# JADGardner/neusky

Measured on AMD Instinct MI355X. Metric: train rays/sec on NeRF-OSR lk2 @1024 rays x 96 samples, higher is better.
Workload: dtype f32 in memory; forward products: fp16 hi + residual split, 3 x v_mfma_f32_32x32x16_f16 per product on power-of-two pre-scaled operands, one fp32 accumulator (~2^-22): FiLM-SIREN chains and the SDF / albedo field alike; backward products: the same fp16 split on per-row / per-matrix pre-scaled gradien; 1 GPU; full NeuSky train step (BASELINE configs[2]): 1024 rays/GPU x 96 samples, proposal 256+96, 512 illumination directions (256 upper-hemisphere DDF queries/ray), illumination decoder = this project's FiLM-SIREN H = 128 (RENI-shaped: latent 100x3; the reference's configured Attention decoder is absent from its tree), hash L16 F2 T2^19 x2, 256-wide MLPs; fwd + losses + bwd + all-reduce + 5 Adam groups; rays_per_gpu=1024, samples_per_ray=96, illumination_directions=512, parallelism=ray-sharded dp1, launcher=self-spawned, launch=HIP graph replay (1 graph/step + all-reduce + 5 Adam launches)

## Files before the change

### neusky_amd/csrc/wgrad_native.hip

```cpp
#include "common.h"
#include "../../include/neusky_hip.h"

namespace {

typedef _Float16 f16x8 __attribute__((ext_vector_type(8)));
typedef float f32x16 __attribute__((ext_vector_type(16)));
typedef float f32x4 __attribute__((ext_vector_type(4)));
typedef short s16x4 __attribute__((__vector_size__(4 * sizeof(short))));
typedef __attribute__((address_space(3))) s16x4 lds_s16x4;

struct WgradProblem {
  const float* A;
  const float* B;
  float* dW;
  float* db;
  const float* a_scale_max;
  float b_scale;
  const float* b_scale_max;
  int nnt_a, nnt_b, ldw;
  int tile0;
  int lda, ldb;
  int wa, wb;
  int bias_rows;
  int bias_mod;
};
struct WgradArgs {
  WgradProblem p[NSKY_WGRAD_MAX_PROBLEMS];
  int n_problems, rows, row_blocks, blocks_per_split, n_tiles;
};

__device__ __forceinline__ float pow2_scale(float m, float& inv) {
  if (!(m > 0.0f) || !(m < 3.0e38f)) { inv = 1.0f; return 1.0f; }
  int e;
  (void)frexpf(m, &e);
  e = max(-100, min(100, e));
  inv = ldexpf(1.0f, e - 15);
  return ldexpf(1.0f, 15 - e);
}

__device__ __forceinline__ int xcd_contiguous(int id, int total) {
  const int xcd = id & 7, idx = id >> 3, per = total >> 3, rem = total & 7;
  return xcd * per + min(xcd, rem) + idx;
}

template <bool BF>
__device__ __forceinline__ f32x16 mma(f16x8 x, f16x8 y, f32x16 acc) {
  typedef __bf16 b16x8 __attribute__((ext_vector_type(8)));
  if (BF) return __builtin_amdgcn_mfma_f32_32x32x16_bf16(__builtin_bit_cast(b16x8, x), __builtin_bit_cast(b16x8, y), acc, 0, 0, 0);
  return __builtin_amdgcn_mfma_f32_32x32x16_f16(x, y, acc, 0, 0, 0);
}

template <int WM, int WN, int TM, int TN, bool RM>
__global__ __launch_bounds__(64 * WM * WN, WM * WN == 8 ? 1 : 2) void wgrad_native_kernel(WgradArgs a) {
  constexpr int NW = WM * WN;
  constexpr int NT = NW;
  static_assert(WM * TM == NT && WN * TN == NT, "square output block");
  constexpr int OPB = NT * 4096;
  constexpr int STAGE = 2 * OPB;
  extern __shared__ __attribute__((aligned(16))) unsigned char smem[];

  const int tid = threadIdx.x, lane = tid & 63, wave = tid >> 6;
  const int wm = wave / WN, wn = wave % WN;
  const int logical = xcd_contiguous(blockIdx.x, gridDim.x);
  const int gtile = logical % a.n_tiles, split = logical / a.n_tiles;
  int pi = 0;
  while (pi + 1 < a.n_problems && gtile >= a.p[pi + 1].tile0) ++pi;
  const WgradProblem& P = a.p[pi];
  const int tile = gtile - P.tile0;
  const int kblocks = P.nnt_b / NT;
  const int nb = tile / kblocks, kb = tile % kblocks;
  const int r_beg = split * a.blocks_per_split;
  const int r_end = min(a.row_blocks, r_beg + a.blocks_per_split);
  if (r_beg >= r_end) return;

  float a_inv = 1.0f;
  const float a_scale = P.a_scale_max ? pow2_scale(*P.a_scale_max, a_inv) : 1.0f;
  float b_unused;
  const float b_scale = P.b_scale_max ? pow2_scale(*P.b_scale_max, b_unused) : P.b_scale;
  const bool clamp_b = P.b_scale_max == nullptr;

  const int c = lane & 31, hh = lane >> 5;
  const int rq = lane >> 3, fq = lane & 7;
  const int fa = (nb * NT + wave) * 32 + 4 * fq, fb = (kb * NT + wave) * 32 + 4 * fq;
  const bool fa_ok = fa < P.wa, fb_ok = fb < P.wb;
  const float* pa = RM ? P.A + (long)r_beg * 32 * P.lda + min(fa, max(P.wa - 4, 0))
                       : P.A + ((long)r_beg * P.nnt_a + nb * NT + wave) * 1024 + lane * 4;
  const float* pb = RM ? P.B + (long)r_beg * 32 * P.ldb + min(fb, max(P.wb - 4, 0))
                       : P.B + ((long)r_beg * P.nnt_b + kb * NT + wave) * 1024 + lane * 4;
  const long a_step = RM ? 32l * P.lda : (long)P.nnt_a * 1024, b_step = RM ? 32l * P.ldb : (long)P.nnt_b * 1024;
  int rm_row0 = 0;
  f32x4 raw[8];
  const float* pa2 = pa;
  const float* pb2 = pb;
  auto reload = [&](int uu) {
    if (RM) {
      const int row = min(rm_row0 + 8 * (uu >> 1) + rq, a.rows - 1) - rm_row0;
      raw[uu] = __builtin_nontemporal_load(reinterpret_cast<const f32x4*>(((uu & 1) ? pb2 + (long)row * P.ldb : pa2 + (long)row * P.lda)));
    } else {
      raw[uu] = __builtin_nontemporal_load(reinterpret_cast<const f32x4*>(((uu & 1) ? pb2 : pa2) + (uu >> 1) * 256));
    }
  };
  float bias[4][4];
#pragma unroll
  for (int u = 0; u < 4; ++u)
#pragma unroll
    for (int i = 0; i < 4; ++i) bias[u][i] = 0.0f;
  const bool want_bias = P.db != nullptr && kb == 0;
  const int w_base = wave * 4096 + c * 64 + 8 * hh;
  const int w_swz = (c >> 1) & 3;
  typedef _Float16 f16x4 __attribute__((ext_vector_type(4)));
  typedef __bf16 b16x4 __attribute__((ext_vector_type(4)));
  auto stage_unit = [&](int uu, int row0, bool row_block_live, unsigned char* stage) {
    const int op = uu & 1, u = uu >> 1;
    const float s = op == 0 ? a_scale : b_scale;
    const int row = row0 + (RM ? 8 * u + rq : c);
    const bool live = row_block_live && row < a.rows && (!RM || (op == 0 ? fa_ok : fb_ok));
    const bool bias_on = op == 0 && row < P.bias_rows && (P.bias_mod <= 1 || (row % P.bias_mod) == 0);
    float v[4];
#pragma unroll
    for (int i = 0; i < 4; ++i) {
      v[i] = live ? raw[uu][i] * s : 0.0f;
      if (op == 1 && clamp_b) v[i] = __builtin_amdgcn_fmed3f(v[i], -65504.0f, 65504.0f);
      if (op == 0) bias[u][i] += bias_on ? v[i] : 0.0f;
    }
    unsigned char* img;
    if (RM) {
      const int r = 8 * u + rq;
      img = stage + op * OPB + wave * 4096 + r * 64 + 16 * ((fq >> 1) ^ ((r >> 1) & 3)) + 8 * (fq & 1);
      b16x4 h4, l4;
#pragma unroll
      for (int i = 0; i < 4; ++i) { h4[i] = (__bf16)v[i]; l4[i] = (__bf16)(v[i] - (float)h4[i]); }
      *reinterpret_cast<b16x4*>(img) = h4;
      *reinterpret_cast<b16x4*>(img + 2048) = l4;
    } else {
      img = stage + op * OPB + w_base + 16 * (u ^ w_swz);
      f16x4 h4, l4;
#pragma unroll
      for (int i = 0; i < 4; ++i) { h4[i] = (_Float16)v[i]; l4[i] = (_Float16)(v[i] - (float)h4[i]); }
      *reinterpret_cast<f16x4*>(img) = h4;
      *reinterpret_cast<f16x4*>(img + 2048) = l4;
    }
  };

  const int i16 = lane & 15, q = i16 >> 2, p = i16 & 3, gsel = (lane >> 4) & 1, h = lane >> 5;
  int t_off[2];
#pragma unroll
  for (int rd = 0; rd < 2; ++rd) {
    const int row = 8 * h + 4 * rd + q;
    t_off[rd] = row * 64 + 16 * ((2 * gsel + (p >> 1)) ^ ((row >> 1) & 3)) + 8 * (p & 1);
  }
  auto frag = [&](const unsigned char* img, int ks) -> f16x8 {
    const s16x4 lo4 = __builtin_amdgcn_ds_read_tr16_b64_v4i16((lds_s16x4*)(img + ks * 1024 + t_off[0]));
    const s16x4 hi4 = __builtin_amdgcn_ds_read_tr16_b64_v4i16((lds_s16x4*)(img + ks * 1024 + t_off[1]));
    typedef short s16x8 __attribute__((ext_vector_type(8)));
    const s16x8 v = {lo4[0], lo4[1], lo4[2], lo4[3], hi4[0], hi4[1], hi4[2], hi4[3]};
    return __builtin_bit_cast(f16x8, v);
  };

  f32x16 acc[TM][TN];
#pragma unroll
  for (int i = 0; i < TM; ++i)
#pragma unroll
    for (int j = 0; j < TN; ++j)
#pragma unroll
      for (int r = 0; r < 16; ++r) acc[i][j][r] = 0.0f;

  rm_row0 = r_beg * 32;
#pragma unroll
  for (int uu = 0; uu < 8; ++uu) reload(uu);
  {
    if (r_beg + 1 < r_end) { pa2 += a_step; pb2 += b_step; rm_row0 += 32; }
#pragma unroll
    for (int uu = 0; uu < 8; ++uu) {
      stage_unit(uu, r_beg * 32, true, smem);
      reload(uu);
    }
    if (r_beg + 2 < r_end) { pa2 += a_step; pb2 += b_step; rm_row0 += 32; }
  }
  static_assert(TN == 4 || TN == 2, "one staging unit per (k-step, X tile) point, or two");
  constexpr int UPP = 8 / (2 * TN);
  int cur = 0;
  for (int r = r_beg; r < r_end; ++r) {
    __syncthreads();
    const bool live = r + 1 < r_end;
    const unsigned char* st = smem + cur * STAGE;
    unsigned char* nxt = smem + (cur ^ 1) * STAGE;
#pragma unroll
    for (int ks = 0; ks < 2; ++ks) {
      f16x8 ah[TM], al[TM], bh[2], bl[2];
#pragma unroll
      for (int i = 0; i < TM; ++i) {
        ah[i] = frag(st + (wm * TM + i) * 4096, ks);
        al[i] = frag(st + (wm * TM + i) * 4096 + 2048, ks);
      }
      bh[0] = frag(st + OPB + (wn * TN) * 4096, ks);
      bl[0] = frag(st + OPB + (wn * TN) * 4096 + 2048, ks);
#pragma unroll
      for (int j = 0; j < TN; ++j) {
        if (j + 1 < TN) {
          bh[(j + 1) & 1] = frag(st + OPB + (wn * TN + j + 1) * 4096, ks);
          bl[(j + 1) & 1] = frag(st + OPB + (wn * TN + j + 1) * 4096 + 2048, ks);
        }
#pragma unroll
        for (int i = 0; i < TM; ++i) acc[i][j] = mma<RM>(al[i], bh[j & 1], acc[i][j]);
#pragma unroll
        for (int i = 0; i < TM; ++i) acc[i][j] = mma<RM>(ah[i], bl[j & 1], acc[i][j]);
#pragma unroll
        for (int i = 0; i < TM; ++i) acc[i][j] = mma<RM>(ah[i], bh[j & 1], acc[i][j]);
#pragma unroll
        for (int k = 0; k < UPP; ++k) {
          const int uu = (ks * TN + j) * UPP + k;
          stage_unit(uu, (r + 1) * 32, live, nxt);
          reload(uu);
        }
        __builtin_amdgcn_sched_barrier(0);
      }
    }
    if (r + 3 < r_end) { pa2 += a_step; pb2 += b_step; rm_row0 += 32; }
    cur ^= 1;
  }

  const float out_scale = a_inv / b_scale;
  const int n0 = (nb * NT + wm * TM) * 32, k0 = (kb * NT + wn * TN) * 32;
#pragma unroll
  for (int i = 0; i < TM; ++i)
#pragma unroll
    for (int j = 0; j < TN; ++j) {
      float* out = P.dW + (long)(n0 + 32 * i + 4 * h) * P.ldw + k0 + 32 * j + (lane & 31);
      const bool col_ok = k0 + 32 * j + (lane & 31) < P.wb;
#pragma unroll
      for (int g = 0; g < 16; ++g)
        if (col_ok && n0 + 32 * i + 4 * h + 8 * (g >> 2) + (g & 3) < P.wa)
          atomicAdd(out + (long)(8 * (g >> 2) + (g & 3)) * P.ldw, acc[i][j][g] * out_scale);
      __builtin_amdgcn_sched_barrier(0);
    }
  if (want_bias && RM) {
#pragma unroll
    for (int i = 0; i < 4; ++i) {
      float v = (bias[0][i] + bias[1][i]) + (bias[2][i] + bias[3][i]);
#pragma unroll
      for (int off = 8; off < 64; off <<= 1) v += __shfl_xor(v, off, 64);
      if (rq == 0 && fa + i < P.wa) atomicAdd(P.db + fa + i, v * a_inv);
    }
  } else if (want_bias) {
#pragma unroll
    for (int u = 0; u < 4; ++u)
#pragma unroll
      for (int i = 0; i < 4; ++i) {
        float v = bias[u][i];
#pragma unroll
        for (int off = 16; off > 0; off >>= 1) v += __shfl_xor(v, off, 64);
        if (c == 0 && (nb * NT + wave) * 32 + 8 * u + 4 * hh + i < P.wa) atomicAdd(P.db + (nb * NT + wave) * 32 + 8 * u + 4 * hh + i, v * a_inv);
      }
  }
}

}

extern "C" int nsky_wgrad_native_batch(const nsky_wgrad_problem* problems, int32_t n_problems, int32_t rows, nsky_stream_t stream) {
  NSKY_CHECK_ARG(problems && n_problems >= 1 && n_problems <= NSKY_WGRAD_MAX_PROBLEMS && rows >= 0,
                 "nsky_wgrad_native_batch: 1..%d problems expected, got %d", NSKY_WGRAD_MAX_PROBLEMS, n_problems);
  if (rows == 0) return NSKY_OK;
  WgradArgs a;
  const bool rm = problems[0].lda > 0;
  bool wide = true;
  for (int i = 0; i < n_problems; ++i) {
    const nsky_wgrad_problem& q = problems[i];
    NSKY_CHECK_ARG(q.dZ && q.X && q.dW, "nsky_wgrad_native_batch: problem %d: null argument", i);
    NSKY_CHECK_ARG((q.lda > 0) == rm && (q.ldb > 0) == rm, "nsky_wgrad_native_batch: problem %d: row-major and tile-native operands in one launch", i);
    if (rm) {
      NSKY_CHECK_ARG(q.width_a >= 4 && q.width_b >= 4 && q.width_a % 4 == 0 && q.width_b % 4 == 0 && q.lda >= q.width_a && q.ldb >= q.width_b &&
                         q.lda % 4 == 0 && q.ldb % 4 == 0, "nsky_wgrad_native_batch: problem %d: row-major widths / leading dimensions must be multiples of 4", i);
      NSKY_CHECK_ARG(q.ldw >= q.width_b && q.a_scale_max == nullptr, "nsky_wgrad_native_batch: problem %d: ldw %d < %d, or a scale with row-major operands", i,
                     q.ldw, q.width_b);
      wide = wide && q.width_a > 128 && q.width_b > 128;
    } else {
      NSKY_CHECK_ARG(q.nnt_a > 0 && q.nnt_b > 0 && q.nnt_a % 4 == 0 && q.nnt_b % 4 == 0,
                     "nsky_wgrad_native_batch: problem %d: both operands need a multiple of 128 features (got %d and %d tiles of 32)", i,
                     q.nnt_a, q.nnt_b);
      NSKY_CHECK_ARG(q.width_a >= 0 && q.width_a <= 32 * q.nnt_a && q.width_b >= 0 && q.width_b <= 32 * q.nnt_b,
                     "nsky_wgrad_native_batch: problem %d: widths %d / %d exceed the tiles", i, q.width_a, q.width_b);
      NSKY_CHECK_ARG(q.ldw >= (q.width_b > 0 ? q.width_b : 32 * q.nnt_b), "nsky_wgrad_native_batch: problem %d: ldw %d too small", i, q.ldw);
      int e = 0;
      NSKY_CHECK_ARG(q.b_scale > 0.0f && frexpf(q.b_scale, &e) == 0.5f, "nsky_wgrad_native_batch: problem %d: b_scale must be a power of two", i);
      wide = wide && q.nnt_a % 8 == 0 && q.nnt_b % 8 == 0;
    }
  }
  const int NT = wide ? 8 : 4;
  int tiles = 0;
  for (int i = 0; i < n_problems; ++i) {
    const nsky_wgrad_problem& q = problems[i];
    WgradProblem& P = a.p[i];
    P.A = q.dZ; P.B = q.X; P.dW = q.dW; P.db = q.db; P.a_scale_max = q.a_scale_max; P.b_scale = rm ? 1.0f : q.b_scale;
    P.b_scale_max = rm ? nullptr : q.b_scale_max;
    P.nnt_a = rm ? ceil_div(q.width_a, 32 * NT) * NT : q.nnt_a;
    P.nnt_b = rm ? ceil_div(q.width_b, 32 * NT) * NT : q.nnt_b;
    P.ldw = q.ldw; P.tile0 = tiles;
    P.lda = q.lda; P.ldb = q.ldb;
    P.wa = (rm || q.width_a > 0) ? q.width_a : 32 * q.nnt_a;
    P.wb = (rm || q.width_b > 0) ? q.width_b : 32 * q.nnt_b;
    P.bias_rows = q.bias_rows > 0 ? q.bias_rows : rows;
    P.bias_mod = rm ? 0 : q.bias_row_mod;
    tiles += (P.nnt_a / NT) * (P.nnt_b / NT);
  }
  a.n_problems = n_problems; a.rows = rows; a.n_tiles = tiles;
  a.row_blocks = ceil_div(rows, 32);
  const int slots = wide ? 256 : 512;
  int splits = slots / a.n_tiles;
  if (splits < 1) splits = 1;
  if (splits > a.row_blocks) splits = a.row_blocks;
  a.blocks_per_split = ceil_div(a.row_blocks, splits);
  splits = ceil_div(a.row_blocks, a.blocks_per_split);
  const dim3 grid(a.n_tiles * splits);
  const size_t smem = 2 * 2 * NT * 4096;
  static bool attr_set = [] {
    (void)hipFuncSetAttribute(reinterpret_cast<const void*>(&wgrad_native_kernel<4, 2, 2, 4, false>), hipFuncAttributeMaxDynamicSharedMemorySize, 160 * 1024);
    (void)hipFuncSetAttribute(reinterpret_cast<const void*>(&wgrad_native_kernel<2, 2, 2, 2, false>), hipFuncAttributeMaxDynamicSharedMemorySize, 160 * 1024);
    (void)hipFuncSetAttribute(reinterpret_cast<const void*>(&wgrad_native_kernel<4, 2, 2, 4, true>), hipFuncAttributeMaxDynamicSharedMemorySize, 160 * 1024);
    (void)hipFuncSetAttribute(reinterpret_cast<const void*>(&wgrad_native_kernel<2, 2, 2, 2, true>), hipFuncAttributeMaxDynamicSharedMemorySize, 160 * 1024);
    return true;
  }();
  (void)attr_set;
  const hipStream_t st = (hipStream_t)stream;
  if (wide && rm) hipLaunchKernelGGL((wgrad_native_kernel<4, 2, 2, 4, true>), grid, dim3(512), smem, st, a);
  else if (wide) hipLaunchKernelGGL((wgrad_native_kernel<4, 2, 2, 4, false>), grid, dim3(512), smem, st, a);
  else if (rm) hipLaunchKernelGGL((wgrad_native_kernel<2, 2, 2, 2, true>), grid, dim3(256), smem, st, a);
  else hipLaunchKernelGGL((wgrad_native_kernel<2, 2, 2, 2, false>), grid, dim3(256), smem, st, a);
  NSKY_CHECK_LAUNCH("nsky_wgrad_native_batch");
  return NSKY_OK;
}

extern "C" int nsky_wgrad_native(const float* dZ, int32_t nnt_a, const float* X, int32_t nnt_b, int32_t rows, float* dW, int32_t ldw,
                                 float* db, const float* a_scale_max, float b_scale, nsky_stream_t stream) {
  nsky_wgrad_problem q = {};
  q.dZ = dZ; q.nnt_a = nnt_a; q.X = X; q.nnt_b = nnt_b; q.dW = dW; q.ldw = ldw; q.db = db; q.a_scale_max = a_scale_max; q.b_scale = b_scale;
  return nsky_wgrad_native_batch(&q, 1, rows, stream);
}
```

Before: 52410 rays/s.

## Triple-buffer wgrad LDS per k-step and prefetch next fragments across barriers

Splits the per-row-block LDS staging into half-block (16-row k-step) slots arranged as a three-slot ring, reducing LDS use from 2x to 1.5x of a full block. Fragments for the next k-step are read from LDS during the last MFMA group of the current step, so LDS reads overlap the matrix math. The global-load lane mapping and bias reduction are reorganised to match the new layout. This adds one barrier per k-step, where there was one per row block, and holds more fragment registers live, in exchange for hiding LDS read latency.

```diff
diff --git a/neusky_amd/csrc/wgrad_native.hip b/neusky_amd/csrc/wgrad_native.hip
--- a/neusky_amd/csrc/wgrad_native.hip
+++ b/neusky_amd/csrc/wgrad_native.hip
@@ -55,8 +55,8 @@
   constexpr int NW = WM * WN;
   constexpr int NT = NW;
   static_assert(WM * TM == NT && WN * TN == NT, "square output block");
-  constexpr int OPB = NT * 4096;
-  constexpr int STAGE = 2 * OPB;
+  constexpr int OPB = NT * 2048;
+  constexpr int SLOT = 2 * OPB;
   extern __shared__ __attribute__((aligned(16))) unsigned char smem[];
 
   const int tid = threadIdx.x, lane = tid & 63, wave = tid >> 6;
@@ -79,66 +79,68 @@
   const float b_scale = P.b_scale_max ? pow2_scale(*P.b_scale_max, b_unused) : P.b_scale;
   const bool clamp_b = P.b_scale_max == nullptr;
 
-  const int c = lane & 31, hh = lane >> 5;
+  const int kr = (lane & 7) + 8 * ((lane >> 4) & 1), hh = (lane >> 3) & 1, ug = lane >> 5;
   const int rq = lane >> 3, fq = lane & 7;
   const int fa = (nb * NT + wave) * 32 + 4 * fq, fb = (kb * NT + wave) * 32 + 4 * fq;
   const bool fa_ok = fa < P.wa, fb_ok = fb < P.wb;
+  const int lane_off = ug * 256 + hh * 128 + kr * 4;
   const float* pa = RM ? P.A + (long)r_beg * 32 * P.lda + min(fa, max(P.wa - 4, 0))
-                       : P.A + ((long)r_beg * P.nnt_a + nb * NT + wave) * 1024 + lane * 4;
+                       : P.A + ((long)r_beg * P.nnt_a + nb * NT + wave) * 1024 + lane_off;
   const float* pb = RM ? P.B + (long)r_beg * 32 * P.ldb + min(fb, max(P.wb - 4, 0))
-                       : P.B + ((long)r_beg * P.nnt_b + kb * NT + wave) * 1024 + lane * 4;
+                       : P.B + ((long)r_beg * P.nnt_b + kb * NT + wave) * 1024 + lane_off;
   const long a_step = RM ? 32l * P.lda : (long)P.nnt_a * 1024, b_step = RM ? 32l * P.ldb : (long)P.nnt_b * 1024;
   int rm_row0 = 0;
   f32x4 raw[8];
   const float* pa2 = pa;
   const float* pb2 = pb;
   auto reload = [&](int uu) {
+    const int ks = uu >> 2, v = (uu >> 1) & 1, op = uu & 1;
     if (RM) {
-      const int row = min(rm_row0 + 8 * (uu >> 1) + rq, a.rows - 1) - rm_row0;
-      raw[uu] = __builtin_nontemporal_load(reinterpret_cast<const f32x4*>(((uu & 1) ? pb2 + (long)row * P.ldb : pa2 + (long)row * P.lda)));
+      const int row = min(rm_row0 + 16 * ks + 8 * v + rq, a.rows - 1) - rm_row0;
+      raw[uu] = __builtin_nontemporal_load(reinterpret_cast<const f32x4*>((op ? pb2 + (long)row * P.ldb : pa2 + (long)row * P.lda)));
     } else {
-      raw[uu] = __builtin_nontemporal_load(reinterpret_cast<const f32x4*>(((uu & 1) ? pb2 : pa2) + (uu >> 1) * 256));
+      raw[uu] = __builtin_nontemporal_load(reinterpret_cast<const f32x4*>((op ? pb2 : pa2) + v * 512 + ks * 64));
     }
   };
-  float bias[4][4];
-#pragma unroll
-  for (int u = 0; u < 4; ++u)
-#pragma unroll
-    for (int i = 0; i < 4; ++i) bias[u][i] = 0.0f;
+  float bias[2][4];
+#pragma unroll
+  for (int v = 0; v < 2; ++v)
+#pragma unroll
+    for (int i = 0; i < 4; ++i) bias[v][i] = 0.0f;
   const bool want_bias = P.db != nullptr && kb == 0;
-  const int w_base = wave * 4096 + c * 64 + 8 * hh;
-  const int w_swz = (c >> 1) & 3;
+  const int bias_rows = P.bias_rows, bias_mod = max(P.bias_mod, 1);
+  const bool mod_by_lane = 16 % bias_mod == 0;
+  const bool lane_mod_ok = (RM ? rq : kr) % bias_mod == 0;
   typedef _Float16 f16x4 __attribute__((ext_vector_type(4)));
   typedef __bf16 b16x4 __attribute__((ext_vector_type(4)));
-  auto stage_unit = [&](int uu, int row0, bool row_block_live, unsigned char* stage) {
-    const int op = uu & 1, u = uu >> 1;
+  auto stage_unit = [&](int uu, int row0, bool row_block_live, unsigned char* slot) {
+    const int ks = uu >> 2, v = (uu >> 1) & 1, op = uu & 1;
     const float s = op == 0 ? a_scale : b_scale;
-    const int row = row0 + (RM ? 8 * u + rq : c);
+    const int kro = RM ? 8 * v + rq : kr;
+    const int row = row0 + 16 * ks + kro;
     const bool live = row_block_live && row < a.rows && (!RM || (op == 0 ? fa_ok : fb_ok));
-    const bool bias_on = op == 0 && row < P.bias_rows && (P.bias_mod <= 1 || (row % P.bias_mod) == 0);
-    float v[4];
+    const bool bias_on = op == 0 && row < bias_rows && (mod_by_lane ? lane_mod_ok : row % bias_mod == 0);
+    float x[4];
 #pragma unroll
     for (int i = 0; i < 4; ++i) {
-      v[i] = live ? raw[uu][i] * s : 0.0f;
-      if (op == 1 && clamp_b) v[i] = __builtin_amdgcn_fmed3f(v[i], -65504.0f, 65504.0f);
-      if (op == 0) bias[u][i] += bias_on ? v[i] : 0.0f;
-    }
-    unsigned char* img;
+      x[i] = live ? raw[uu][i] * s : 0.0f;
+      if (op == 1 && clamp_b) x[i] = __builtin_amdgcn_fmed3f(x[i], -65504.0f, 65504.0f);
+      if (op == 0) bias[v][i] += bias_on ? x[i] : 0.0f;
+    }
+    unsigned char* img = slot + op * OPB + wave * 2048 + kro * 64 + 8 * (RM ? (fq & 1) : hh) +
+                         16 * ((RM ? fq >> 1 : 2 * v + ug) ^ ((kro >> 1) & 3));
     if (RM) {
-      const int r = 8 * u + rq;
-      img = stage + op * OPB + wave * 4096 + r * 64 + 16 * ((fq >> 1) ^ ((r >> 1) & 3)) + 8 * (fq & 1);
       b16x4 h4, l4;
 #pragma unroll
-      for (int i = 0; i < 4; ++i) { h4[i] = (__bf16)v[i]; l4[i] = (__bf16)(v[i] - (float)h4[i]); }
+      for (int i = 0; i < 4; ++i) { h4[i] = (__bf16)x[i]; l4[i] = (__bf16)(x[i] - (float)h4[i]); }
       *reinterpret_cast<b16x4*>(img) = h4;
-      *reinterpret_cast<b16x4*>(img + 2048) = l4;
+      *reinterpret_cast<b16x4*>(img + 1024) = l4;
     } else {
-      img = stage + op * OPB + w_base + 16 * (u ^ w_swz);
       f16x4 h4, l4;
 #pragma unroll
-      for (int i = 0; i < 4; ++i) { h4[i] = (_Float16)v[i]; l4[i] = (_Float16)(v[i] - (float)h4[i]); }
+      for (int i = 0; i < 4; ++i) { h4[i] = (_Float16)x[i]; l4[i] = (_Float16)(x[i] - (float)h4[i]); }
       *reinterpret_cast<f16x4*>(img) = h4;
-      *reinterpret_cast<f16x4*>(img + 2048) = l4;
+      *reinterpret_cast<f16x4*>(img + 1024) = l4;
     }
   };
 
@@ -149,9 +151,9 @@
     const int row = 8 * h + 4 * rd + q;
     t_off[rd] = row * 64 + 16 * ((2 * gsel + (p >> 1)) ^ ((row >> 1) & 3)) + 8 * (p & 1);
   }
-  auto frag = [&](const unsigned char* img, int ks) -> f16x8 {
-    const s16x4 lo4 = __builtin_amdgcn_ds_read_tr16_b64_v4i16((lds_s16x4*)(img + ks * 1024 + t_off[0]));
-    const s16x4 hi4 = __builtin_amdgcn_ds_read_tr16_b64_v4i16((lds_s16x4*)(img + ks * 1024 + t_off[1]));
+  auto frag = [&](const unsigned char* img) -> f16x8 {
+    const s16x4 lo4 = __builtin_amdgcn_ds_read_tr16_b64_v4i16((lds_s16x4*)(img + t_off[0]));
+    const s16x4 hi4 = __builtin_amdgcn_ds_read_tr16_b64_v4i16((lds_s16x4*)(img + t_off[1]));
     typedef short s16x8 __attribute__((ext_vector_type(8)));
     const s16x8 v = {lo4[0], lo4[1], lo4[2], lo4[3], hi4[0], hi4[1], hi4[2], hi4[3]};
     return __builtin_bit_cast(f16x8, v);
@@ -172,34 +174,43 @@
     if (r_beg + 1 < r_end) { pa2 += a_step; pb2 += b_step; rm_row0 += 32; }
 #pragma unroll
     for (int uu = 0; uu < 8; ++uu) {
-      stage_unit(uu, r_beg * 32, true, smem);
+      stage_unit(uu, r_beg * 32, true, smem + (uu >> 2) * SLOT);
       reload(uu);
     }
     if (r_beg + 2 < r_end) { pa2 += a_step; pb2 += b_step; rm_row0 += 32; }
   }
   static_assert(TN == 4 || TN == 2, "one staging unit per (k-step, X tile) point, or two");
-  constexpr int UPP = 8 / (2 * TN);
-  int cur = 0;
+  constexpr int UPP = 4 / TN;
+  int s_cur = 0, s_nxt = SLOT, s_wr = 2 * SLOT;
+  f16x8 ah[TM], al[TM], bh[2], bl[2];
+  __syncthreads();
+#pragma unroll
+  for (int i = 0; i < TM; ++i) {
+    ah[i] = frag(smem + (wm * TM + i) * 2048);
+    al[i] = frag(smem + (wm * TM + i) * 2048 + 1024);
+  }
+  bh[0] = frag(smem + OPB + (wn * TN) * 2048);
+  bl[0] = frag(smem + OPB + (wn * TN) * 2048 + 1024);
   for (int r = r_beg; r < r_end; ++r) {
-    __syncthreads();
     const bool live = r + 1 < r_end;
-    const unsigned char* st = smem + cur * STAGE;
-    unsigned char* nxt = smem + (cur ^ 1) * STAGE;
 #pragma unroll
     for (int ks = 0; ks < 2; ++ks) {
-      f16x8 ah[TM], al[TM], bh[2], bl[2];
-#pragma unroll
-      for (int i = 0; i < TM; ++i) {
-        ah[i] = frag(st + (wm * TM + i) * 4096, ks);
-        al[i] = frag(st + (wm * TM + i) * 4096 + 2048, ks);
-      }
-      bh[0] = frag(st + OPB + (wn * TN) * 4096, ks);
-      bl[0] = frag(st + OPB + (wn * TN) * 4096 + 2048, ks);
+      const unsigned char* st = smem + s_cur;
+      const unsigned char* sn = smem + s_nxt;
+      f16x8 nah[TM], nal[TM];
 #pragma unroll
       for (int j = 0; j < TN; ++j) {
         if (j + 1 < TN) {
-          bh[(j + 1) & 1] = frag(st + OPB + (wn * TN + j + 1) * 4096, ks);
-          bl[(j + 1) & 1] = frag(st + OPB + (wn * TN + j + 1) * 4096 + 2048, ks);
+          bh[(j + 1) & 1] = frag(st + OPB + (wn * TN + j + 1) * 2048);
+          bl[(j + 1) & 1] = frag(st + OPB + (wn * TN + j + 1) * 2048 + 1024);
+        } else {
+#pragma unroll
+          for (int i = 0; i < TM; ++i) {
+            nah[i] = frag(sn + (wm * TM + i) * 2048);
+            nal[i] = frag(sn + (wm * TM + i) * 2048 + 1024);
+          }
+          bh[(j + 1) & 1] = frag(sn + OPB + (wn * TN) * 2048);
+          bl[(j + 1) & 1] = frag(sn + OPB + (wn * TN) * 2048 + 1024);
         }
 #pragma unroll
         for (int i = 0; i < TM; ++i) acc[i][j] = mma<RM>(al[i], bh[j & 1], acc[i][j]);
@@ -209,15 +220,19 @@
         for (int i = 0; i < TM; ++i) acc[i][j] = mma<RM>(ah[i], bh[j & 1], acc[i][j]);
 #pragma unroll
         for (int k = 0; k < UPP; ++k) {
-          const int uu = (ks * TN + j) * UPP + k;
-          stage_unit(uu, (r + 1) * 32, live, nxt);
+          const int uu = 4 * ks + j * UPP + k;
+          stage_unit(uu, (r + 1) * 32, live, smem + s_wr);
           reload(uu);
         }
         __builtin_amdgcn_sched_barrier(0);
       }
+#pragma unroll
+      for (int i = 0; i < TM; ++i) { ah[i] = nah[i]; al[i] = nal[i]; }
+      const int s_old = s_cur;
+      s_cur = s_nxt; s_nxt = s_wr; s_wr = s_old;
+      __syncthreads();
     }
     if (r + 3 < r_end) { pa2 += a_step; pb2 += b_step; rm_row0 += 32; }
-    cur ^= 1;
   }
 
   const float out_scale = a_inv / b_scale;
@@ -237,20 +252,22 @@
   if (want_bias && RM) {
 #pragma unroll
     for (int i = 0; i < 4; ++i) {
-      float v = (bias[0][i] + bias[1][i]) + (bias[2][i] + bias[3][i]);
+      float v = bias[0][i] + bias[1][i];
 #pragma unroll
       for (int off = 8; off < 64; off <<= 1) v += __shfl_xor(v, off, 64);
       if (rq == 0 && fa + i < P.wa) atomicAdd(P.db + fa + i, v * a_inv);
     }
   } else if (want_bias) {
 #pragma unroll
-    for (int u = 0; u < 4; ++u)
+    for (int v = 0; v < 2; ++v)
 #pragma unroll
       for (int i = 0; i < 4; ++i) {
-        float v = bias[u][i];
-#pragma unroll
-        for (int off = 16; off > 0; off >>= 1) v += __shfl_xor(v, off, 64);
-        if (c == 0 && (nb * NT + wave) * 32 + 8 * u + 4 * hh + i < P.wa) atomicAdd(P.db + (nb * NT + wave) * 32 + 8 * u + 4 * hh + i, v * a_inv);
+        float x = bias[v][i];
+#pragma unroll
+        for (int off = 1; off < 32; off <<= 1)
+          if (off != 8) x += __shfl_xor(x, off, 64);
+        const int f = (nb * NT + wave) * 32 + 8 * (2 * v + ug) + 4 * hh + i;
+        if ((lane & 0x17) == 0 && f < P.wa) atomicAdd(P.db + f, x * a_inv);
       }
   }
 }
@@ -312,7 +329,7 @@
   a.blocks_per_split = ceil_div(a.row_blocks, splits);
   splits = ceil_div(a.row_blocks, a.blocks_per_split);
   const dim3 grid(a.n_tiles * splits);
-  const size_t smem = 2 * 2 * NT * 4096;
+  const size_t smem = 3 * 2 * NT * 2048;
   static bool attr_set = [] {
     (void)hipFuncSetAttribute(reinterpret_cast<const void*>(&wgrad_native_kernel<4, 2, 2, 4, false>), hipFuncAttributeMaxDynamicSharedMemorySize, 160 * 1024);
     (void)hipFuncSetAttribute(reinterpret_cast<const void*>(&wgrad_native_kernel<2, 2, 2, 2, false>), hipFuncAttributeMaxDynamicSharedMemorySize, 160 * 1024);
```

After: 53860 rays/s (median of 6 runs). 2.8% higher.
